# Xharlie/BtcDet

Hardware: AMD Instinct MI355X
Metric: scenes/s fwd+bwd KITTI-Car bs=2/GPU (BtcDet hot path) (higher is better)
Workload: dtype f32

## Files before the change

btcdet_amd/csrc/btc_common.h:

```cpp
#pragma once
#include <hip/hip_runtime.h>
#include <stdint.h>
#include <stdio.h>

#include "../../include/btcdet_hip.h"

#define BTC_EMPTY_KEY (-1)
#define BTC_EMPTY_IDX 0x7F7F7F7F

void btc_set_error(const char* fmt, ...);

#define BTC_CHECK_ARG(cond, ...)            \
  do {                                      \
    if (!(cond)) {                          \
      btc_set_error(__VA_ARGS__);           \
      return BTC_EINVAL;                    \
    }                                       \
  } while (0)

#define BTC_HIP(call)                                                             \
  do {                                                                            \
    hipError_t e_ = (call);                                                       \
    if (e_ != hipSuccess) {                                                       \
      btc_set_error("%s failed: %s (%s:%d)", #call, hipGetErrorString(e_), __FILE__, __LINE__); \
      return BTC_ELAUNCH;                                                         \
    }                                                                             \
  } while (0)

#define BTC_LAUNCH_CHECK()                                                        \
  do {                                                                            \
    hipError_t e_ = hipGetLastError();                                            \
    if (e_ != hipSuccess) {                                                       \
      btc_set_error("kernel launch failed: %s (%s:%d)", hipGetErrorString(e_), __FILE__, __LINE__); \
      return BTC_ELAUNCH;                                                         \
    }                                                                             \
  } while (0)

#if defined(__HIP_DEVICE_COMPILE__) && !defined(__gfx950__)
#error "the fence-free last-arriver protocol (btc_ticket_take) is derived for gfx950's sc1 write-through stores only"
#endif
#if defined(__HIPCC__)
template <class T>
__device__ __forceinline__ void btc_st_agent(T* p, T v) { __hip_atomic_store(p, v, __ATOMIC_RELAXED, __HIP_MEMORY_SCOPE_AGENT); }
template <class T>
__device__ __forceinline__ T btc_ld_agent(const T* p) { return __hip_atomic_load(p, __ATOMIC_RELAXED, __HIP_MEMORY_SCOPE_AGENT); }
__device__ __forceinline__ int btc_ticket_take(int32_t* counter) {
  asm volatile("s_waitcnt vmcnt(0)" ::: "memory");
  return __hip_atomic_fetch_add(counter, 1, __ATOMIC_RELAXED, __HIP_MEMORY_SCOPE_AGENT);
}
__device__ __forceinline__ void btc_ticket_acquire() { __builtin_amdgcn_fence(__ATOMIC_ACQUIRE, "agent"); }
__device__ __forceinline__ bool btc_last_arriver(int32_t* counter, int total) {
  __shared__ int s_last;
  asm volatile("s_waitcnt vmcnt(0)" ::: "memory");
  __syncthreads();
  if (threadIdx.x == 0) s_last = (btc_ticket_take(counter) == total - 1);
  __syncthreads();
  if (!s_last) return false;
  if (threadIdx.x == 0) btc_ticket_acquire();
  __syncthreads();
  return true;
}
#endif

#define BTC_TUNE_KEYS 24
int btc_tune_get(int key);

bool btc_apply_glds_supported(int K, int Cred, int Cres);
bool btc_apply_glds_has_shape(int shape, bool bf = false);
size_t btc_apply_glds_lds_bytes(int shape, int kc, int K, bool bf, int stages = 3);
int btc_apply_glds_stages(int shape, int kc, int K, bool bf, int asked);
int btc_launch_apply_glds(bool trans_w, int shape, int kc, int xcd, bool bf, const void* feat, const float* W, const float* bias,
                          const int32_t* nbr, const int32_t* order , int n_rows, int K, int Cred, int Cres, void* out,
                          hipStream_t stream, const struct BnFuse* bn = nullptr );

int btc_apply(const char* who, int pass, int operands, const void* src, long long src_rows, const void* W, const float* bias, const int32_t* nbr,
              const int32_t* order, int n_rows, int K, int Cin, int Cout, void* dst, hipStream_t stream, const struct BnFuse* bn);

int btc_apply_bf16w(const void* src, const void* Wq, const float* bias, const int32_t* nbr, const int32_t* order, int n_rows, int K, int Cred,
                    int Cres, void* dst, hipStream_t stream, int mirror = 0, const struct BnFuse* bn = nullptr);
constexpr size_t BTC_SCRATCH_HEAD = 64 * 1024;
constexpr long long BTC_SCRATCH_TICKETS = BTC_SCRATCH_HEAD / 4;
void* btc_scratch(hipStream_t stream, size_t* bytes);
struct BnFuse;
int btc_apply_split(const float* src, const void* Ws, const float* bias, const int32_t* nbr, const int32_t* order, int n_rows, int K, int Cred,
                    int Cres, float* dst, hipStream_t stream, int mirror, const BnFuse* bn);

__host__ __device__ __forceinline__ unsigned short btc_f32_to_bf16(float f) {
  union { float f; unsigned u; } c;
  c.f = f;
  unsigned u = c.u;
  if ((u & 0x7fffffffu) > 0x7f800000u) return (unsigned short)((u >> 16) | 0x40);
  u += 0x7fffu + ((u >> 16) & 1u);
  return (unsigned short)(u >> 16);
}
__host__ __device__ __forceinline__ float btc_bf16_to_f32(unsigned short h) {
  union { float f; unsigned u; } c;
  c.u = (unsigned)h << 16;
  return c.f;
}

template <bool BF>
__device__ __forceinline__ float4 btc_ld4(const float* base, size_t i) {
  if (!BF) return *reinterpret_cast<const float4*>(base + i);
  const uint2 v = *reinterpret_cast<const uint2*>(reinterpret_cast<const unsigned short*>(base) + i);
  return make_float4(__uint_as_float(v.x << 16), __uint_as_float(v.x & 0xffff0000u), __uint_as_float(v.y << 16),
                     __uint_as_float(v.y & 0xffff0000u));
}
template <bool BF>
__device__ __forceinline__ float btc_ld1(const float* base, size_t i) {
  if (!BF) return base[i];
  return __uint_as_float((unsigned)reinterpret_cast<const unsigned short*>(base)[i] << 16);
}
template <bool BF>
__device__ __forceinline__ void btc_st4(float* base, size_t i, float a, float b, float c, float d) {
  if (!BF) {
    *reinterpret_cast<float4*>(base + i) = make_float4(a, b, c, d);
  } else {
    uint2 v;
    v.x = (unsigned)btc_f32_to_bf16(a) | ((unsigned)btc_f32_to_bf16(b) << 16);
    v.y = (unsigned)btc_f32_to_bf16(c) | ((unsigned)btc_f32_to_bf16(d) << 16);
    *reinterpret_cast<uint2*>(reinterpret_cast<unsigned short*>(base) + i) = v;
  }
}
template <bool BF>
__device__ __forceinline__ void btc_st1(float* base, size_t i, float a) {
  if (!BF) base[i] = a;
  else reinterpret_cast<unsigned short*>(base)[i] = btc_f32_to_bf16(a);
}

#ifdef __cplusplus
#include <mutex>
constexpr int BTC_MAX_DEVICES = 16;
struct BtcPerDeviceOnce {
  std::once_flag flag[BTC_MAX_DEVICES];
};
template <class F>
static inline void btc_once_per_device(BtcPerDeviceOnce& o, F&& fn) {
  int dev = 0;
  (void)hipGetDevice(&dev);
  std::call_once(o.flag[dev >= 0 && dev < BTC_MAX_DEVICES ? dev : 0], fn);
}
#endif

typedef float f32x4 __attribute__((ext_vector_type(4)));
constexpr int TM = 64;
__host__ __device__ constexpr int ldb_of(int nt) { return nt * 16 + (((nt * 16) % 32 == 0) ? 16 : 0); }

static inline int btc_cdiv(long long a, long long b) { return (int)((a + b - 1) / b); }
static inline size_t btc_align(size_t x, size_t a = 256) { return (x + a - 1) / a * a; }
static inline unsigned btc_pow2_ge(unsigned long long v) {
  unsigned long long p = 1;
  while (p < v) p <<= 1;
  return (unsigned)p;
}

struct BtcCarver {
// ... 35 lines not shown
```

btcdet_amd/csrc/conv_apply_glds.hip:

```cpp
#include "conv_tile.h"

namespace {

__device__ float g_zero_row[64];

constexpr int G_STAGES_DEFAULT = 3;
constexpr int G_STAGES_MAX = 8;

__device__ __forceinline__ void transpose4(const f32x4 v, float& y0, float& y1, float& y2, float& y3) {
  unsigned x0 = __float_as_uint(v[0]), x1 = __float_as_uint(v[1]), x2 = __float_as_uint(v[2]), x3 = __float_as_uint(v[3]);
  auto a = __builtin_amdgcn_permlane32_swap(x0, x2, false, false);
  x0 = a[0]; x2 = a[1];
  auto b = __builtin_amdgcn_permlane32_swap(x1, x3, false, false);
  x1 = b[0]; x3 = b[1];
  auto c = __builtin_amdgcn_permlane16_swap(x0, x1, false, false);
  x0 = c[0]; x1 = c[1];
  auto d = __builtin_amdgcn_permlane16_swap(x2, x3, false, false);
  x2 = d[0]; x3 = d[1];
  y0 = __uint_as_float(x0); y1 = __uint_as_float(x1); y2 = __uint_as_float(x2); y3 = __uint_as_float(x3);
}

template <int WR, int WC, int NTW, bool TRANS_W, int KC, bool BF>
__global__ __launch_bounds__(64 * WR * WC) void conv_apply_g(const void* __restrict__ feat_, const float* __restrict__ W,
                                                             const float* __restrict__ bias, const int32_t* __restrict__ nbr,
// ... 98 lines not shown
      const float* B = (const float*)(ring + st * STAGE + A_BYTES);
      const int aswz = ((wr * 16 + arow) / RPB) & (UPR - 1);
      constexpr int Q = KC / 4;
      constexpr int G = (16 / NTW) < 1 ? 1 : ((16 / NTW) > Q ? Q : (16 / NTW));
      constexpr int NGRP = Q / G;
      float a[2][G], b[2][G][NTW];
      constexpr bool A128 = !BF && (G % 4 == 0);
      constexpr bool B128 = TRANS_W && (G % 4 == 0) && UPB >= 8 && NTW == 1;
      auto load_group = [&](int g, int buf) {
        if (A128) {
#pragma unroll
          for (int jb = 0; jb < G / 4; ++jb) {
            const int u = (g * (G / 4) + jb) * 4 + kq;
            const f32x4 v = *(const f32x4*)(A + ((u ^ aswz) * 16));
            transpose4(v, a[buf][4 * jb], a[buf][4 * jb + 1], a[buf][4 * jb + 2], a[buf][4 * jb + 3]);
          }
        }
        if (B128) {
#pragma unroll
          for (int nt = 0; nt < NTW; ++nt) {
            const float* colp = B + ((wc * NTW + nt) * 16 + arow) * KC;
#pragma unroll
            for (int jb = 0; jb < G / 4; ++jb) {
              const int u = (g * (G / 4) + jb) * 4 + kq;
              const f32x4 v = *(const f32x4*)(colp + ((u ^ (arow & (UPB - 1))) * 4));
              transpose4(v, b[buf][4 * jb][nt], b[buf][4 * jb + 1][nt], b[buf][4 * jb + 2][nt], b[buf][4 * jb + 3][nt]);
            }
          }
        }
#pragma unroll
        for (int i = 0; i < G; ++i) {
          const int q = g * G + i;
          if (A128) {
          } else if (!BF) {
            a[buf][i] = *(const float*)(A + ((q ^ aswz) * 16) + kq * 4);
          } else {
            const unsigned short h = *(const unsigned short*)(A + (((q >> 1) ^ aswz) * 16) + (((q & 1) * 4 + kq) * 2));
            a[buf][i] = __uint_as_float((unsigned)h << 16);
          }
          if (!TRANS_W) {
            const float* bp = B + (q * 4 + kq) * TN + arow;
#pragma unroll
            for (int nt = 0; nt < NTW; ++nt) {
              const int cg = wc * NTW + nt;
              b[buf][i][nt] = bp[((NG >= 2) ? (cg ^ (kq & 1)) : cg) * 16];
            }
          } else if (!B128) {
            const float* bp = B + (wc * NTW * 16 + arow) * KC + (q ^ (arow & (UPB - 1))) * 4 + kq;
#pragma unroll
            for (int nt = 0; nt < NTW; ++nt) b[buf][i][nt] = bp[nt * 16 * KC];
          }
        }
      };
      load_group(0, 0);
#pragma unroll
      for (int g = 0; g < NGRP; ++g) {
        if (g + 1 < NGRP) load_group(g + 1, (g + 1) & 1);
        __builtin_amdgcn_sched_barrier(0);
#pragma unroll
        for (int i = 0; i < G; ++i)
#pragma unroll
          for (int nt = 0; nt < NTW; ++nt)
            acc[nt] = __builtin_amdgcn_mfma_f32_16x16x4f32(a[g & 1][i], b[g & 1][i][nt], acc[nt], 0, 0, 0);
        __builtin_amdgcn_sched_barrier(0);
      }
    }
    st = (st == S - 1) ? 0 : st + 1;
  }

  float vals[NTW][4];
  bool valid[4];
  int rows[4];
#pragma unroll
  for (int r = 0; r < 4; ++r) rows[r] = s_row[wr * 16 + kq * 4 + r];
  const bool ev = !TRANS_W && bn.ev_mean != nullptr;
  typedef typename std::conditional<BF, unsigned short, float>::type OUT;
  apply_tile_epilogue<NTW>(acc, rows, n0 + wc * NTW * 16, bias, Cres, (OUT*)out_, bn, ev, vals, valid);
  if (bn.slots) {
    bn_fuse_wave<NTW>(bn, vals, valid, n0 + wc * NTW * 16, (int)((bx * WR + wr) & (bn.nslots - 1)));
    bn_fuse_finish(bn, (int*)smem, (double*)(smem + 16));
  }
}

template <int WR, int WC, int NTW, bool TRANS_W, int KC, bool BF>
int launch_g(const void* feat, const float* W, const float* bias, const int32_t* nbr, const int32_t* order, int n_rows, int K, int Cred,
             int Cres, void* out, int xcd, hipStream_t stream, const BnFuse& bn) {
  constexpr int TM = 16 * WR, TN = 16 * NTW * WC;
  const int stages = btc_apply_glds_stages(WR * 100 + WC * 10 + NTW, KC, K, BF, (xcd >> APPLY_STAGES_SHIFT) & 15);
  xcd = (xcd & (APPLY_XCD | APPLY_MIRROR)) | (stages << APPLY_STAGES_SHIFT);
  const size_t lds = btc_apply_glds_lds_bytes(WR * 100 + WC * 10 + NTW, KC, K, BF, stages);
  return apply_launch<conv_apply_g<WR, WC, NTW, TRANS_W, KC, BF>>("conv_apply_g", dim3(btc_cdiv(n_rows, TM), Cres / TN), 64 * WR * WC, lds, stream, feat, W,
                                                                  bias, nbr, order, n_rows, K, Cred, Cres, out, xcd,
                                                                  btc_tune_get(BTC_TUNE_APPLY_DEBUG), bn);
}

#define G_ARGS feat, W, bias, nbr, order, n_rows, K, Cred, Cres, out, xcd, stream, bn
#define G_PARAMS                                                                                                             \
  const void *feat, const float *W, const float *bias, const int32_t *nbr, const int32_t *order, int n_rows, int K, int Cred, int Cres, \
      void *out, int xcd, hipStream_t stream, const BnFuse &bn

template <int WR, int WC, int NTW, bool TRANS_W, bool BF>
int launch_g_kc(int kc, G_PARAMS) {
  switch (kc) {
    case 16: return launch_g<WR, WC, NTW, TRANS_W, 16, BF>(G_ARGS);
    case 32: return launch_g<WR, WC, NTW, TRANS_W, 32, BF>(G_ARGS);
    default: return launch_g<WR, WC, NTW, TRANS_W, 64, BF>(G_ARGS);
  }
}

template <bool TRANS_W>
int launch_g_shape(int wr, int wc, int ntw, int kc, bool bf, G_PARAMS) {
  const int code = wr * 100 + wc * 10 + ntw;
  switch (code) {
#define G_CASE2(WR_, WC_, NTW_)                                                      \
  case WR_ * 100 + WC_ * 10 + NTW_:                                                  \
    return bf ? launch_g_kc<WR_, WC_, NTW_, TRANS_W, true>(kc, G_ARGS) : launch_g_kc<WR_, WC_, NTW_, TRANS_W, false>(kc, G_ARGS)
#define G_CASE(WR_, WC_, NTW_)      \
  case WR_ * 100 + WC_ * 10 + NTW_: \
    if (bf) break;                  \
    return launch_g_kc<WR_, WC_, NTW_, TRANS_W, false>(kc, G_ARGS)
    G_CASE2(4, 1, 1); G_CASE(4, 1, 2); G_CASE(4, 1, 4); G_CASE(4, 1, 8);
    G_CASE(4, 2, 1); G_CASE2(4, 2, 2); G_CASE2(4, 2, 4);
    G_CASE2(2, 2, 1); G_CASE(2, 2, 2); G_CASE(2, 2, 4);
    G_CASE(2, 4, 1); G_CASE(2, 4, 2);
    G_CASE2(1, 4, 1); G_CASE(1, 4, 2);
#undef G_CASE
#undef G_CASE2
    default: break;
  }
  btc_set_error("conv_apply_g: no instance for WR=%d WC=%d NTW=%d bf16=%d", wr, wc, ntw, (int)bf);
  return BTC_EINVAL;
}

}

bool btc_apply_glds_has_shape(int shape, bool bf) {
  static const int shapes[] = {411, 412, 414, 418, 421, 422, 424, 221, 222, 224, 241, 242, 141, 142};
  static const int shapes_bf[] = {411, 422, 424, 221, 141};
  if (bf) {
    for (int v : shapes_bf)
      if (v == shape) return true;
    return false;
  }
  for (int v : shapes)
    if (v == shape) return true;
  return false;
}

size_t btc_apply_glds_lds_bytes(int shape, int kc, int K, bool bf, int stages) {
  const int tm = 16 * (shape / 100), tn = 16 * ((shape / 10) % 10) * (shape % 10);
  const size_t a_bytes = ((size_t)tm * kc * (bf ? 2 : 4) + 1023) / 1024 * 1024;
  return (size_t)(stages > 0 ? stages : G_STAGES_DEFAULT) * (a_bytes + (size_t)kc * tn * 4) + apply_tail_bytes(tm, K);
}

int btc_apply_glds_stages(int shape, int kc, int K, bool bf, int asked) {
  const int tm = 16 * (shape / 100), tn = 16 * ((shape / 10) % 10) * (shape % 10), nw = (shape / 100) * ((shape / 10) % 10);
  const size_t a_bytes = ((size_t)tm * kc * (bf ? 2 : 4) + 1023) / 1024 * 1024, stage = a_bytes + (size_t)kc * tn * 4;
  const int npi = (int)(((a_bytes / 1024) + nw - 1) / nw + ((size_t)kc * tn / 256 + nw - 1) / nw);
  int s = asked ? asked : btc_tune_get(BTC_TUNE_APPLY_STAGES);
  if (!s) {
    s = (int)((size_t)48 * 1024 / stage);
    if (s > 6) s = 6;
  }
  if (s < 3) s = 3;
  if (s > G_STAGES_MAX) s = G_STAGES_MAX;
  while (s > 3 && ((s - 2) * npi > 63 || btc_apply_glds_lds_bytes(shape, kc, K, bf, s) > 160 * 1024)) --s;
  return s;
}

bool btc_apply_glds_supported(int K, int Cred, int Cres) { return K <= 64 && Cred % 16 == 0 && Cres % 16 == 0 && Cred >= 16; }

int btc_launch_apply_glds(bool trans_w, int shape, int kc, int xcd, bool bf, const void* feat, const float* W, const float* bias,
                          const int32_t* nbr, const int32_t* order, int n_rows, int K, int Cred, int Cres, void* out, hipStream_t stream,
                          const BnFuse* bn_) {
  if (n_rows <= 0) return BTC_OK;
  const BnFuse bn = bn_ ? *bn_ : btc_bn_fuse_none();
  const int wr = shape / 100, wc = (shape / 10) % 10, ntw = shape % 10;
  BTC_CHECK_ARG(btc_apply_glds_supported(K, Cred, Cres) && wc * ntw > 0 && Cres % (16 * wc * ntw) == 0 && Cred % kc == 0 &&
                    (kc == 16 || kc == 32 || kc == 64),
                "conv_apply_g: unsupported K=%d Cred=%d Cres=%d shape=%d kc=%d", K, Cred, Cres, shape, kc);
  return trans_w ? launch_g_shape<true>(wr, wc, ntw, kc, bf, G_ARGS) : launch_g_shape<false>(wr, wc, ntw, kc, bf, G_ARGS);
}
```

btcdet_amd/csrc/sparse_conv.hip:

```cpp
#include "conv_tile.h"

namespace {

constexpr int KC = 32;
constexpr int LDA = KC + 2;

template <int NT, bool TRANS_W, bool VEC, int KB, int THREADS>
__global__ __launch_bounds__(THREADS) void conv_apply(const float* __restrict__ feat, const float* __restrict__ W,
                                                  const float* __restrict__ bias, const int32_t* __restrict__ nbr,
                                                  int n_rows, int K, int Cred, int Cres, float* __restrict__ out, int mirror, const BnFuse bn) {
  extern __shared__ __attribute__((aligned(16))) char smem[];
  constexpr int TM = THREADS / 4;
  constexpr int LDB = ldb_of(NT);
  constexpr int NB = NT * 512 / THREADS;
  float* As = (float*)smem;
  float* Bs = As + KB * TM * LDA;
  int32_t* s_nbr = (int32_t*)(Bs + KB * KC * LDB);
  int32_t* s_kact = s_nbr + TM * K;
  int32_t* s_nact = s_kact + K;

  const int tid = threadIdx.x, lane = tid & 63, wave = tid >> 6;
  const int row0 = blockIdx.x * TM;
  const int n0 = blockIdx.y * (NT * 16);

// ... 251 lines not shown
    constexpr bool ev = EV;
#pragma unroll
    for (int r = 0; r < 4; ++r) valid[r] = row0 + kq * 4 + r < n_rows;
#pragma unroll
    for (int nt = 0; nt < NT; ++nt) {
      const int col = nt * 16 + lrow;
      const float bv0 = (bias && col < Cres) ? bias[col] : 0.f;
      BnEvalCol ec = {0.f, 0.f, 1.f, 0.f};
      if (ev) ec = bn_eval_col(bn, col);
#pragma unroll
      for (int r = 0; r < 4; ++r) {
        const int row = row0 + kq * 4 + r;
        vals[nt][r] = bias ? (acc[nt][r] + bv0) : acc[nt][r];
        if (ev) vals[nt][r] = bn_affine(vals[nt][r], ec.m, ec.rs, ec.g, ec.b, bn.ev_relu);
        if (col < Cres && row < n_rows) out[(size_t)row * Cres + col] = vals[nt][r];
      }
    }
    if (bn.slots) bn_fuse_wave<NT>(bn, vals, valid, 0, (int)(tile & (bn.nslots - 1)));
    __builtin_amdgcn_wave_barrier();
  }
  if (bn.slots) bn_fuse_finish(bn, (int*)smem, (double*)(smem + 16));
}


__global__ __launch_bounds__(256) void maxpool_fwd_k(const float* __restrict__ feat, const int32_t* __restrict__ nbr,
                                                     int n_out, int K, int C, float* __restrict__ out) {
  long long t = (long long)blockIdx.x * blockDim.x + threadIdx.x;
  if (t >= (long long)n_out * C) return;
  int i = (int)(t / C), c = (int)(t % C);
  float m = 0.f;
  for (int k = 0; k < K; ++k) {
    int j = nbr[(size_t)i * K + k];
    if (j >= 0) m = fmaxf(m, feat[(size_t)j * C + c]);
  }
  out[t] = m;
}

__global__ __launch_bounds__(256) void maxpool_bwd_k(const float* __restrict__ feat, const float* __restrict__ out,
                                                     const float* __restrict__ dout, const int32_t* __restrict__ nbr_in,
                                                     int n_in, int K, int C, float* __restrict__ din) {
  long long t = (long long)blockIdx.x * blockDim.x + threadIdx.x;
  if (t >= (long long)n_in * C) return;
  int j = (int)(t / C), c = (int)(t % C);
  float v = feat[t], g = 0.f;
  for (int k = 0; k < K; ++k) {
    int i = nbr_in[(size_t)j * K + k];
    if (i >= 0 && out[(size_t)i * C + c] == v) g += dout[(size_t)i * C + c];
  }
  din[t] = g;
}

__global__ __launch_bounds__(256) void dense_fwd_k(const float* __restrict__ feat, const int4* __restrict__ idx, int n, int C,
                                                   int D, int H, int Wd, float* __restrict__ dense) {
  long long t = (long long)blockIdx.x * blockDim.x + threadIdx.x;
  if (t >= (long long)n * C) return;
  int c = (int)(t / n), i = (int)(t % n);
  int4 q = idx[i];
  size_t vol = (size_t)D * H * Wd;
  dense[((size_t)q.x * C + c) * vol + ((size_t)q.y * H + q.z) * Wd + q.w] = feat[(size_t)i * C + c];
}

__global__ __launch_bounds__(256) void dense_bwd_k(const float* __restrict__ ddense, const int4* __restrict__ idx, int n, int C,
                                                   int D, int H, int Wd, float* __restrict__ dfeat) {
  long long t = (long long)blockIdx.x * blockDim.x + threadIdx.x;
  if (t >= (long long)n * C) return;
  int c = (int)(t / n), i = (int)(t % n);
  int4 q = idx[i];
  size_t vol = (size_t)D * H * Wd;
  dfeat[(size_t)i * C + c] = ddense[((size_t)q.x * C + c) * vol + ((size_t)q.y * H + q.z) * Wd + q.w];
}

template <int NT, bool TRANS_W, int THREADS>
int launch_apply_t(dim3 grid, size_t lds, hipStream_t stream, bool vec, const float* feat, const float* W, const float* bias,
                   const int32_t* nbr, int n_rows, int K, int Cred, int Cres, float* out, int mirror, const BnFuse& bn) {
  if (vec) return apply_launch<conv_apply<NT, TRANS_W, true, 1, THREADS>>("conv_apply", grid, THREADS, lds, stream, feat, W, bias, nbr, n_rows, K, Cred, Cres, out, mirror, bn);
  return apply_launch<conv_apply<NT, TRANS_W, false, 1, THREADS>>("conv_apply", grid, THREADS, lds, stream, feat, W, bias, nbr, n_rows, K, Cred, Cres, out, mirror, bn);
}

template <bool TRANS_W, bool EV>
int launch_ws(int nt, int wgs, size_t lds, hipStream_t stream, const float* feat, const float* W, const float* bias, const int32_t* nbr, int n_rows,
              int K, int Cred, int Cres, float* out, int mirror, const BnFuse& bn) {
  if (nt == 1) return apply_launch<conv_apply_ws<1, TRANS_W, EV>>("conv_apply_ws", wgs, WS_WAVES * 64, lds, stream, feat, W, bias, nbr, n_rows, K, Cred, Cres, out, mirror, bn);
  return apply_launch<conv_apply_ws<2, TRANS_W, EV>>("conv_apply_ws", wgs, WS_WAVES * 64, lds, stream, feat, W, bias, nbr, n_rows, K, Cred, Cres, out, mirror, bn);
}

template <bool TRANS_W>
int launch_apply(const float* feat, const float* W, const float* bias, const int32_t* nbr, int n_rows, int K, int Cred,
                 int Cres, float* out, hipStream_t stream, bool bf = false, const int32_t* order = nullptr, int mirror = 0,
                 const BnFuse* bn_ = nullptr) {
  const BnFuse bn = bn_ ? *bn_ : btc_bn_fuse_none();
  if (n_rows <= 0) return BTC_OK;
  BTC_CHECK_ARG(!bf || btc_apply_glds_supported(K, Cred, Cres),
                "bf16 activations need channel counts that are multiples of 16 (K=%d, %d -> %d): convert to fp32", K, Cred, Cres);
  int nt = Cres <= 16 ? 1 : (Cres <= 32 ? 2 : (Cres <= 64 ? 4 : 8));
  const int t_kernel = btc_tune_get(BTC_TUNE_APPLY_KERNEL), t_nt = btc_tune_get(BTC_TUNE_APPLY_NT);
  if (bf || (t_kernel != 1 && btc_apply_glds_supported(K, Cred, Cres) && (t_kernel == 2 || n_rows < 100000 || (Cred >= 64 && Cres >= 64)))) {
    int shape, kc = (Cred % 64 == 0) ? 64 : ((Cred % 32 == 0) ? 32 : 16);
    if (bf) {
      if (Cres % 128 == 0) shape = 424;
      else if (Cres % 64 == 0) shape = n_rows < 8192 ? 141 : 422;
      else if (Cres % 32 == 0) shape = 221;
      else shape = 411;
    } else if (Cres % 128 == 0) {
      shape = n_rows < 7000 ? 222 : (n_rows < 13000 ? 242 : (n_rows <= 16384 ? 424 : (n_rows < 19500 ? 242 : 424)));
    } else if (Cres % 64 == 0) {
      if (kc == 64) shape = n_rows < 11000 ? 141 : 241;
      else shape = n_rows < 13000 ? 141 : 222;
    } else if (Cres % 32 == 0) {
      shape = 221;
    } else {
      shape = 411;
    }
    if (t_nt > 8 && !bf) {
      int wc = (t_nt / 10) % 10, ntw = t_nt % 10;
      while (ntw > 1 && Cres % (16 * wc * ntw)) ntw >>= 1;
      while (wc > 1 && Cres % (16 * wc * ntw)) wc >>= 1;
      const int cand = (t_nt / 100) * 100 + wc * 10 + ntw;
      if (btc_apply_glds_has_shape(cand)) shape = cand;
    }
    const int t_kc = btc_tune_get(BTC_TUNE_APPLY_KC);
    if (t_kc && Cred % t_kc == 0) kc = t_kc;
    while (kc > 16 && btc_apply_glds_lds_bytes(shape, kc, K, bf) > 160 * 1024) kc >>= 1;
    return btc_launch_apply_glds(TRANS_W, shape, kc, apply_flags(mirror), bf, feat, W, bias, nbr, order, n_rows, K, Cred, Cres, out, stream, &bn);
  }
  if (t_kernel != 1 && Cred <= 4 * WS_Q && Cres <= 32 && K <= 64 && n_rows >= 2048 && ws_lds_bytes(K, Cred, nt) <= 160 * 1024) {
    const int n_tiles16 = btc_cdiv(n_rows, 16);
    int wgs = btc_cdiv(n_tiles16, WS_WAVES);
    if (wgs > 256) wgs = 256;
    size_t lds = ws_lds_bytes(K, Cred, nt);
    if (bn.slots && lds < 16 + (size_t)16 * WS_WAVES * 64) lds = 16 + (size_t)16 * WS_WAVES * 64;
    if constexpr (!TRANS_W) {
      if (bn.ev_mean) return launch_ws<false, true>(nt, wgs, lds, stream, feat, W, bias, nbr, n_rows, K, Cred, Cres, out, mirror, bn);
    }
    return launch_ws<TRANS_W, false>(nt, wgs, lds, stream, feat, W, bias, nbr, n_rows, K, Cred, Cres, out, mirror, bn);
  }
  const int tm = 64;
  const int n_tiles = btc_cdiv(n_rows, tm);
  while (nt > 2 && (long long)n_tiles * btc_cdiv(Cres, nt * 16) < 512) nt >>= 1;
  if (t_nt && t_nt <= 8) nt = t_nt;
  dim3 grid(n_tiles, btc_cdiv(Cres, nt * 16));
  size_t lds = (size_t)(tm * LDA + KC * ldb_of(nt)) * sizeof(float) + (size_t)(tm * K + K + 1) * sizeof(int32_t);
  const bool vec = (Cred & 3) == 0;
#define BTC_APPLY(NT_) launch_apply_t<NT_, TRANS_W, 256>(grid, lds, stream, vec, feat, W, bias, nbr, n_rows, K, Cred, Cres, out, mirror, bn)
  switch (nt) {
    case 1: return BTC_APPLY(1);
    case 2: return BTC_APPLY(2);
    case 4: return BTC_APPLY(4);
    default: return BTC_APPLY(8);
  }
#undef BTC_APPLY
}

int split_source_ok(const char* who, long long src_rows, int Cred) {
  BTC_CHECK_ARG(src_rows >= 0, "%s: BTC_OPERANDS_F32_SPLIT needs the row count of src (btc_conv_apply_src / btc_conv_bn_relu_fwd_src)", who);
  BTC_CHECK_ARG(src_rows * Cred * 4 < 0xFFFFFF00LL, "%s: a source of %lld rows x %d channels is past the 32-bit gather offsets of the split-operand "
                "kernel (4 GB): use BTC_OPERANDS_F32", who, src_rows, Cred);
  return BTC_OK;
}

}

int btc_apply(const char* who, int pass, int operands, const void* src, long long src_rows, const void* W, const float* bias, const int32_t* nbr,
              const int32_t* order, int n_rows, int K, int Cin, int Cout, void* dst, hipStream_t stream, const BnFuse* bn) {
  BTC_CHECK_ARG((pass == BTC_PASS_FWD || pass == BTC_PASS_DGRAD || pass == BTC_PASS_DGRAD_MIRROR) && operands >= BTC_OPERANDS_F32 &&
                    operands <= BTC_OPERANDS_F32_SPLIT, "%s: pass=%d operands=%d", who, pass, operands);
  const int mirror = pass == BTC_PASS_DGRAD_MIRROR;
  const bool fwd = pass == BTC_PASS_FWD;
  BTC_CHECK_ARG(K <= BTC_CONV_K_MAX, "%s: K=%d offsets, more than BTC_CONV_K_MAX = %d", who, K, BTC_CONV_K_MAX);
  BTC_CHECK_ARG(K >= 1 && Cin >= 1 && Cout >= 1 && n_rows >= 0, "%s: bad sizes", who);
  BTC_CHECK_ARG(fwd || bias == nullptr, "%s: dgrad takes no bias", who);
  BTC_CHECK_ARG(!bn || Cout <= BN_FUSE_CMAX, "%s: more than %d channels", who, BN_FUSE_CMAX);
  const int Cred = fwd ? Cin : Cout, Cres = fwd ? Cout : Cin;
  if (operands == BTC_OPERANDS_BF16) {
    const bool ok = btc_conv_bf16w_supported(K, Cred, Cres);
    if (bn) BTC_CHECK_ARG(ok, "%s: bf16 operands need K <= 64, Cin %% 32 == 0, Cout %% 16 == 0", who);
    else BTC_CHECK_ARG(ok, "%s: bf16 operands need K <= 64, Cred %% 32 == 0, Cres %% 16 == 0 (K=%d, %d -> %d)", who, K, Cin, Cout);
    return btc_apply_bf16w(src, W, bias, nbr, order, n_rows, K, Cred, Cres, dst, stream, mirror, bn);
  }
  if (operands == BTC_OPERANDS_F32_SPLIT) {
    if (n_rows > 0) {
      const int rc = split_source_ok(who, src_rows, Cred);
      if (rc) return rc;
    }
    return btc_apply_split((const float*)src, W, bias, nbr, order, n_rows, K, Cred, Cres, (float*)dst, stream, mirror, bn);
  }
  const bool bf = operands == BTC_OPERANDS_BF16_ACT;
  if (fwd) return launch_apply<false>((const float*)src, (const float*)W, bias, nbr, n_rows, K, Cred, Cres, (float*)dst, stream, bf, order, 0, bn);
  return launch_apply<true>((const float*)src, (const float*)W, nullptr, nbr, n_rows, K, Cred, Cres, (float*)dst, stream, bf, order, mirror, bn);
}

#define BTC_SIZES_OK(who, n) BTC_CHECK_ARG(K >= 1 && Cin >= 1 && Cout >= 1 && (n) >= 0, who ": bad sizes")

extern "C" int btc_conv_fwd(const float* feat, const float* W, const float* bias, const int32_t* nbr_out, int n_out, int K,
                            int Cin, int Cout, float* out, void* stream) {
  BTC_SIZES_OK("btc_conv_fwd", n_out);
  return btc_apply("btc_conv_fwd", BTC_PASS_FWD, BTC_OPERANDS_F32, feat, -1LL, W, bias, nbr_out, nullptr, n_out, K, Cin, Cout, out, (hipStream_t)stream, nullptr);
}

extern "C" int btc_conv_dgrad(const float* dout, const float* W, const int32_t* nbr_in, int n_in, int K, int Cin, int Cout,
                              float* din, void* stream) {
  BTC_SIZES_OK("btc_conv_dgrad", n_in);
  return btc_apply("btc_conv_dgrad", BTC_PASS_DGRAD, BTC_OPERANDS_F32, dout, -1LL, W, nullptr, nbr_in, nullptr, n_in, K, Cin, Cout, din, (hipStream_t)stream, nullptr);
}

extern "C" int btc_conv_fwd_bf16(const void* feat, const float* W, const float* bias, const int32_t* nbr_out, int n_out, int K,
                                 int Cin, int Cout, void* out, void* stream) {
// ... 73 lines not shown
```

include/btcdet_hip.h:

```cpp
#ifndef BTCDET_HIP_H
#define BTCDET_HIP_H

#include <stddef.h>
#include <stdint.h>

#ifdef __cplusplus
extern "C" {
#endif

#define BTC_OK 0
#define BTC_EINVAL (-1)
#define BTC_ELAUNCH (-2)
#define BTC_ERANGE (-3)

#define BTC_MODE_SUBM 0
#define BTC_MODE_CONV 1
#define BTC_MODE_TRANSPOSE 2

const char* btc_last_error(void);
int btc_version(void);

#define BTC_TUNE_APPLY_KERNEL 0
#define BTC_TUNE_APPLY_NT 1
#define BTC_TUNE_APPLY_XCD 2
#define BTC_TUNE_APPLY_KC 4
#define BTC_TUNE_WGRAD_PH 5
#define BTC_TUNE_WGRAD_WGS 6
#define BTC_TUNE_POV_SELECT 7
#define BTC_TUNE_BF16_OPERANDS 8
#define BTC_TUNE_BN_FWD_KB 9
#define BTC_TUNE_BN_BWD_KB 10
#define BTC_TUNE_WGRAD_PIPE 11
#define BTC_TUNE_BN_FUSE 12
#define BTC_TUNE_SPLIT_Z 15
#define BTC_TUNE_SPLIT_LOADERS 17
#define BTC_TUNE_SPLIT 14
#define BTC_TUNE_APPLY_STAGES 13
#define BTC_TUNE_WGRAD_X 18
#define BTC_TUNE_WGRAD_X_DEPTH 20
#define BTC_TUNE_RB_MARK_MULTI 19
#define BTC_TUNE_SPLIT_PAIR 21
#define BTC_TUNE_WGRAD_NARROW 22
#define BTC_TUNE_EVAL_FOLD 23
#define BTC_TUNE_APPLY_DEBUG 3
int btc_tune_set(int key, int value);
int btc_tune_value(int key);

size_t btc_voxelize_ws_bytes(int n, int batch, int max_points);
int btc_voxelize(const float* points, int n, int ld, int xyz_col, int feat_col, int C,
                 const int32_t* scene_offsets, int batch, const float* h_range, const float* h_vsize,
                 const int32_t* h_grid, int max_points, int max_voxels, float* voxels, int32_t* coords,
                 int32_t* num, int32_t* d_total, void* ws, size_t ws_bytes, void* stream);

int btc_cart_to_occ_coords(const float* in, float* out, int n, int ld, int mode, void* stream);

int btc_voxel_shift_col(float* voxels, const int32_t* coords, int m, int max_points, int C, int col,
                        const float* rot_by_batch, float sign, void* stream);

size_t btc_range_mask_ws_bytes(int n);
int btc_range_mask_compact(const float* points, const float* points_b, int n, int ld, int ld_b, const int32_t* scene_offsets, int batch,
                           const float* h_range_xyxy, float* out, float* out_b, int32_t* out_offsets, int32_t* keep_idx, void* ws,
                           size_t ws_bytes, void* stream);
int btc_gather_rows(const float* src, const int32_t* idx, int n_out, int ld, int n_src, float* out, int32_t* bad_count, void* stream);

int btc_out_shape(const int32_t* h_in_shape, const int32_t* h_k, const int32_t* h_s, const int32_t* h_p,
                  const int32_t* h_d, const int32_t* h_outpad, int mode, int32_t* h_out_shape);

size_t btc_rulebook_subm_ws_bytes(int n);
int btc_rulebook_subm(const int32_t* indices, int n, int batch, const int32_t* h_shape, const int32_t* h_k,
                      const int32_t* h_d, int32_t* nbr_out, int32_t* nbr_in, void* ws, size_t ws_bytes,
                      void* stream);

size_t btc_rulebook_conv_ws_bytes(int batch, const int32_t* h_out_shape);
int btc_rulebook_conv_count(const int32_t* indices, int n, int batch, const int32_t* h_in_shape,
                            const int32_t* h_out_shape, const int32_t* h_k, const int32_t* h_s,
                            const int32_t* h_p, const int32_t* h_d, int mode, int32_t* d_n_out, void* ws,
                            size_t ws_bytes, void* stream);
int btc_rulebook_conv_fill(const int32_t* indices, int n, int batch, const int32_t* h_in_shape,
                           const int32_t* h_out_shape, const int32_t* h_k, const int32_t* h_s,
                           const int32_t* h_p, const int32_t* h_d, int mode, int n_out, int32_t* out_indices,
                           int32_t* nbr_out, int32_t* nbr_in, void* ws, size_t ws_bytes, void* stream);

#define BTC_CHAIN_MAX_LAYERS 32
typedef struct BtcChainLayer {
  int32_t kind, ref, mode;
  int32_t in_shape[3], out_shape[3], k[3], s[3], p[3], d[3];
} BtcChainLayer;
size_t btc_chain_ws_bytes(const BtcChainLayer* h_layers, int n_layers, int batch, int n0);
int btc_chain_caps(const BtcChainLayer* h_layers, int n_layers, int batch, int n0, int64_t* h_cap);
int btc_chain_levels(const int32_t* indices, int n0, int batch, const BtcChainLayer* h_layers, int n_layers,
                     int32_t* const* h_out_indices, const int64_t* h_cap, int32_t* d_counts, void* ws, size_t ws_bytes, void* stream);
int btc_chain_maps(const int32_t* indices, int n0, int batch, const BtcChainLayer* h_layers, int n_layers, const int32_t* h_counts,
                   int32_t* const* h_out_indices, int32_t* const* h_nbr_out, int32_t* const* h_nbr_in,
                   int32_t* const* h_first_out ,
                   int32_t* const* h_first_in , void* ws, size_t ws_bytes, void* stream);

size_t btc_pairs_from_nbr_ws_bytes(int n_out, int K);
int btc_pairs_from_nbr(const int32_t* nbr_out, int n_out, int K, int n_in, int32_t* pairs, int32_t* pair_num, void* ws,
                       size_t ws_bytes, void* stream);

int btc_conv_fwd(const float* feat, const float* W, const float* bias , const int32_t* nbr_out,
                 int n_out, int K, int Cin, int Cout, float* out, void* stream);
int btc_conv_dgrad(const float* dout, const float* W, const int32_t* nbr_in, int n_in, int K, int Cin,
                   int Cout, float* din, void* stream);
size_t btc_conv_wgrad_ws_bytes(int n_out, int K, int Cin, int Cout, int n_in);
int btc_conv_wgrad(const float* feat, const float* dout, const int32_t* nbr_out, int n_out, const int32_t* nbr_in,
                   int n_in, int K, int Cin, int Cout, float* dW, void* ws, size_t ws_bytes, void* stream);

int btc_conv_fwd_bf16(const void* feat, const float* W, const float* bias, const int32_t* nbr_out, int n_out, int K, int Cin,
                      int Cout, void* out, void* stream);
int btc_conv_dgrad_bf16(const void* dout, const float* W, const int32_t* nbr_in, int n_in, int K, int Cin, int Cout,
                        void* din, void* stream);
int btc_conv_wgrad_bf16(const void* feat, const void* dout, const int32_t* nbr_out, int n_out, const int32_t* nbr_in,
                        int n_in, int K, int Cin, int Cout, float* dW, void* ws, size_t ws_bytes, void* stream);

int btc_conv_bf16w_supported(int K, int Cred, int Cres);
int btc_weights_to_bf16(const float* W, int K, int Cin, int Cout, void* w_bf16, void* wt_bf16, void* stream);
int btc_weights_to_bf16_multi(const float* const* W, void* const* w_bf16, void* const* wt_bf16, const int32_t* K, const int32_t* Cin,
                              const int32_t* Cout, int n, void* stream);
int btc_conv_fwd_bf16w(const void* feat, const void* wt_bf16, const float* bias, const int32_t* nbr_out, int n_out, int K, int Cin,
                       int Cout, void* out, void* stream);
int btc_conv_dgrad_bf16w(const void* dout, const void* w_bf16, const int32_t* nbr_in, int n_in, int K, int Cin, int Cout, void* din,
                         void* stream);

// ... 209 lines not shown
```

Before: 583.8.

## Batch several kernel offsets per pipeline item in gather-LDS conv apply

Adds a conv_apply_gk kernel variant in which each pipeline stage loads KB kernel offsets' activation rows and weights at once when the reduced channel count fits in a single chunk (Cred == kc ≤ 32, fp32 activations). The aim is to cut the number of per-item waits and barriers and to give each stage more MFMA work for narrow-channel layers. By default it picks KB=4 for kc=16 and KB=2 for kc=32 on the supported tile shapes, and a new tune key can override this. The cost is larger LDS stages, which may lower occupancy or the number of stages, plus extra template instances.

Result: no change. 582.1 (-0.3%).

```diff
diff --git a/btcdet_amd/csrc/btc_common.h b/btcdet_amd/csrc/btc_common.h
--- a/btcdet_amd/csrc/btc_common.h
+++ b/btcdet_amd/csrc/btc_common.h
@@ -67,11 +67,13 @@
 
 bool btc_apply_glds_supported(int K, int Cred, int Cres);
 bool btc_apply_glds_has_shape(int shape, bool bf = false);
-size_t btc_apply_glds_lds_bytes(int shape, int kc, int K, bool bf, int stages = 3);
-int btc_apply_glds_stages(int shape, int kc, int K, bool bf, int asked);
+bool btc_apply_glds_has_kb(int shape, int kc, int kb);
+size_t btc_apply_glds_lds_bytes(int shape, int kc, int K, bool bf, int stages = 3, int kb = 1);
+int btc_apply_glds_stages(int shape, int kc, int K, bool bf, int asked, int kb = 1);
 int btc_launch_apply_glds(bool trans_w, int shape, int kc, int xcd, bool bf, const void* feat, const float* W, const float* bias,
                           const int32_t* nbr, const int32_t* order , int n_rows, int K, int Cred, int Cres, void* out,
-                          hipStream_t stream, const struct BnFuse* bn = nullptr );
+                          hipStream_t stream, const struct BnFuse* bn = nullptr ,
+                          int kb = 1 );
 
 int btc_apply(const char* who, int pass, int operands, const void* src, long long src_rows, const void* W, const float* bias, const int32_t* nbr,
               const int32_t* order, int n_rows, int K, int Cin, int Cout, void* dst, hipStream_t stream, const struct BnFuse* bn);
diff --git a/btcdet_amd/csrc/conv_apply_glds.hip b/btcdet_amd/csrc/conv_apply_glds.hip
--- a/btcdet_amd/csrc/conv_apply_glds.hip
+++ b/btcdet_amd/csrc/conv_apply_glds.hip
@@ -204,13 +204,219 @@
   }
 }
 
-template <int WR, int WC, int NTW, bool TRANS_W, int KC, bool BF>
+template <int WR, int WC, int NTW, bool TRANS_W, int KC, bool BF, int KB>
+__global__ __launch_bounds__(64 * WR * WC) void conv_apply_gk(const void* __restrict__ feat_, const float* __restrict__ W,
+                                                             const float* __restrict__ bias, const int32_t* __restrict__ nbr,
+                                                             const int32_t* __restrict__ order, int n_rows, int K, int Cred, int Cres,
+                                                             void* __restrict__ out_, int flags, int dbg, const BnFuse bn) {
+  extern __shared__ __attribute__((aligned(16))) char smem[];
+  const int S = ((flags >> APPLY_STAGES_SHIFT) & 15) ? ((flags >> APPLY_STAGES_SHIFT) & 15) : G_STAGES_DEFAULT;
+  constexpr int NW = WR * WC, THREADS = 64 * NW;
+  constexpr int TM = 16 * WR, TN = 16 * NTW * WC, NG = NTW * WC;
+  constexpr int ES = BF ? 2 : 4;
+  constexpr int KW = KB * KC;
+  static_assert(KW <= 64 && (KB == 1 || !BF), "an item is 64 channels at most; several offsets per item: fp32 activations");
+  constexpr int UPR = KW * ES / 16;
+  constexpr int UPS = KC * ES / 16;
+  constexpr int UPB = KW / 4;
+  constexpr int RPB = (128 / (KW * ES)) < 1 ? 1 : (128 / (KW * ES));
+  constexpr int A_UNITS = TM * UPR;
+  constexpr int NAI_TOTAL = (A_UNITS + 63) / 64;
+  constexpr int NAI = (NAI_TOTAL + NW - 1) / NW;
+  constexpr int NBI_TOTAL = KW * TN / 256;
+  constexpr int NBI = (NBI_TOTAL + NW - 1) / NW;
+  constexpr int NPI = NAI + NBI;
+  constexpr int A_BYTES = (TM * KW * ES + 1023) / 1024 * 1024;
+  constexpr int STAGE = A_BYTES + KW * TN * 4;
+  char* ring = smem;
+  APPLY_TAIL(ring + S * STAGE, TM, K);
+  const char* feat = (const char*)feat_;
+
+  const int tid = threadIdx.x, lane = tid & 63, wave = tid >> 6;
+  const int wr = wave / WC, wc = wave % WC;
+  const ApplyTile tile = apply_tile_prologue<TM, THREADS>(s_nbr, s_kact, s_nact, s_row, nbr, order, n_rows, K, flags, wr);
+  const int bx = tile.bx, n0 = blockIdx.y * TN, n_act = tile.n_act;
+  const unsigned long long wave_act = tile.wave_act;
+  const int n_chunks = Cred / KC;
+  const int n_items = (dbg & 32) ? 0 : (KB > 1 ? (n_act + KB - 1) / KB : n_act * n_chunks);
+  if (dbg & 16) return;
+  f32x4 acc[NTW];
+#pragma unroll
+  for (int nt = 0; nt < NTW; ++nt) acc[nt] = (f32x4){0.f, 0.f, 0.f, 0.f};
+
+  int iq = 0, ir = 0, cq = 0, cr = 0;
+  auto issue = [&](int st) {
+    const int k = s_kact[iq];
+    const int cc = ir * KC;
+    const int ib = iq, last = n_act - 1;
+    if constexpr (KB > 1) iq += KB;
+    else if (++ir == n_chunks) { ir = 0; ++iq; }
+    char* As = ring + st * STAGE;
+    float* Bs = (float*)(As + A_BYTES);
+#pragma unroll
+    for (int t = 0; t < NAI; ++t) {
+      if (dbg & 8) break;
+      const int ai = (wave + NW * t) % NAI_TOTAL;
+      const int U = ai * 64 + lane;
+      if (A_UNITS % 64 == 0 || U < A_UNITS) {
+        const int rloc = U / UPR;
+        const int uw = (U % UPR) ^ ((rloc / RPB) & (UPR - 1));
+        const int e = ib + uw / UPS, u = uw % UPS;
+        int nb;
+        if constexpr (KB == 1) nb = s_nbr[rloc * K + k];
+        else nb = e <= last ? s_nbr[rloc * K + s_kact[e]] : -1;
+        const char* src = nb >= 0 ? feat + ((size_t)nb * Cred + cc) * ES + u * 16 : (const char*)g_zero_row;
+        glds16(src, As + ai * 1024);
+      }
+    }
+    const float* Wk1 = W + (size_t)k * Cred * Cres;
+#pragma unroll
+    for (int t = 0; t < NBI; ++t) {
+      if (dbg & 4) break;
+      const int ii = (wave + NW * t) % NBI_TOTAL;
+      const int U = ii * 64 + lane;
+      const float* src;
+      if (!TRANS_W) {
+        const int kw = U / (TN / 4), pu = U % (TN / 4);
+        const int e = ib + kw / KC, kr = kw % KC;
+        const float* Wk = KB == 1 ? Wk1 : W + (size_t)s_kact[e <= last ? e : last] * Cred * Cres;
+        const int g = (NG >= 2) ? ((pu >> 2) ^ (kr & 1)) : (pu >> 2);
+        src = Wk + (size_t)(cc + kr) * Cres + n0 + g * 16 + (pu & 3) * 4;
+      } else {
+        const int c = U / UPB, pu = U % UPB;
+        const int rw = pu ^ (c & (UPB - 1));
+        const int e = ib + rw / (KC / 4), ru = rw % (KC / 4);
+        const float* Wk = KB == 1 ? Wk1 : W + (size_t)s_kact[e <= last ? e : last] * Cred * Cres;
+        src = Wk + (size_t)(n0 + c) * Cred + cc + ru * 4;
+      }
+      glds16(src, Bs + ii * 256);
+    }
+  };
+
+  const int arow = lane & 15, kq = lane >> 4;
+#define WAIT_ITEMS(n) wait_vm<((n) * NPI > 63 ? 63 : (n) * NPI)>()
+  for (int i = 0; i < S - 1 && i < n_items; ++i) issue(i);
+  int st = 0;
+  for (int item = 0; item < n_items; ++item) {
+    const int left = n_items - 1 - item, fl = left < S - 2 ? left : S - 2;
+    switch (fl) {
+      case 0: wait_vm<0>(); break;
+      case 1: WAIT_ITEMS(1); break;
+      case 2: WAIT_ITEMS(2); break;
+      case 3: WAIT_ITEMS(3); break;
+      case 4: WAIT_ITEMS(4); break;
+      case 5: WAIT_ITEMS(5); break;
+      default: WAIT_ITEMS(6); break;
+    }
+#undef WAIT_ITEMS
+    __builtin_amdgcn_s_barrier();
+    asm volatile("" ::: "memory");
+    if (item + S - 1 < n_items && !(dbg & 2)) issue(st == 0 ? S - 1 : st - 1);
+    const int k0 = s_kact[cq], cb = cq;
+    if constexpr (KB > 1) cq += KB;
+    else if (++cr == n_chunks) { cr = 0; ++cq; }
+#pragma unroll
+    for (int sb = 0; sb < KB; ++sb) {
+      if (KB > 1 && cb + sb >= n_act) break;
+      const int k = sb == 0 ? k0 : s_kact[cb + sb];
+      if (((wave_act >> k) & 1ull) && !(dbg & 1)) {
+        const char* A = ring + st * STAGE + (wr * 16 + arow) * (KW * ES);
+        const float* B = (const float*)(ring + st * STAGE + A_BYTES);
+        const int aswz = ((wr * 16 + arow) / RPB) & (UPR - 1);
+        const int ua = sb * UPS, ub = sb * (KC / 4);
+        constexpr int Q = KC / 4;
+        constexpr int G = (16 / NTW) < 1 ? 1 : ((16 / NTW) > Q ? Q : (16 / NTW));
+        constexpr int NGRP = Q / G;
+        float a[2][G], b[2][G][NTW];
+        constexpr bool A128 = !BF && (G % 4 == 0);
+        constexpr bool B128 = TRANS_W && (G % 4 == 0) && UPB >= 8 && NTW == 1;
+        auto load_group = [&](int g, int buf) {
+          if (A128) {
+#pragma unroll
+            for (int jb = 0; jb < G / 4; ++jb) {
+              const int u = (g * (G / 4) + jb) * 4 + kq;
+              const f32x4 v = *(const f32x4*)(A + (((ua + u) ^ aswz) * 16));
+              transpose4(v, a[buf][4 * jb], a[buf][4 * jb + 1], a[buf][4 * jb + 2], a[buf][4 * jb + 3]);
+            }
+          }
+          if (B128) {
+#pragma unroll
+            for (int nt = 0; nt < NTW; ++nt) {
+              const float* colp = B + ((wc * NTW + nt) * 16 + arow) * KW;
+#pragma unroll
+              for (int jb = 0; jb < G / 4; ++jb) {
+                const int u = (g * (G / 4) + jb) * 4 + kq;
+                const f32x4 v = *(const f32x4*)(colp + (((ub + u) ^ (arow & (UPB - 1))) * 4));
+                transpose4(v, b[buf][4 * jb][nt], b[buf][4 * jb + 1][nt], b[buf][4 * jb + 2][nt], b[buf][4 * jb + 3][nt]);
+              }
+            }
+          }
+#pragma unroll
+          for (int i = 0; i < G; ++i) {
+            const int q = g * G + i;
+            if (A128) {
+            } else if (!BF) {
+              a[buf][i] = *(const float*)(A + (((ua + q) ^ aswz) * 16) + kq * 4);
+            } else {
+              const unsigned short h = *(const unsigned short*)(A + (((ua + (q >> 1)) ^ aswz) * 16) + (((q & 1) * 4 + kq) * 2));
+              a[buf][i] = __uint_as_float((unsigned)h << 16);
+            }
+            if (!TRANS_W) {
+              const float* bp = B + (sb * KC + q * 4 + kq) * TN + arow;
+#pragma unroll
+              for (int nt = 0; nt < NTW; ++nt) {
+                const int cg = wc * NTW + nt;
+                b[buf][i][nt] = bp[((NG >= 2) ? (cg ^ (kq & 1)) : cg) * 16];
+              }
+            } else if (!B128) {
+              const float* bp = B + (wc * NTW * 16 + arow) * KW + ((ub + q) ^ (arow & (UPB - 1))) * 4 + kq;
+#pragma unroll
+              for (int nt = 0; nt < NTW; ++nt) b[buf][i][nt] = bp[nt * 16 * KW];
+            }
+          }
+        };
+        load_group(0, 0);
+#pragma unroll
+        for (int g = 0; g < NGRP; ++g) {
+          if (g + 1 < NGRP) load_group(g + 1, (g + 1) & 1);
+          __builtin_amdgcn_sched_barrier(0);
+#pragma unroll
+          for (int i = 0; i < G; ++i)
+#pragma unroll
+            for (int nt = 0; nt < NTW; ++nt)
+              acc[nt] = __builtin_amdgcn_mfma_f32_16x16x4f32(a[g & 1][i], b[g & 1][i][nt], acc[nt], 0, 0, 0);
+          __builtin_amdgcn_sched_barrier(0);
+        }
+      }
+    }
+    st = (st == S - 1) ? 0 : st + 1;
+  }
+
+  float vals[NTW][4];
+  bool valid[4];
+  int rows[4];
+#pragma unroll
+  for (int r = 0; r < 4; ++r) rows[r] = s_row[wr * 16 + kq * 4 + r];
+  const bool ev = !TRANS_W && bn.ev_mean != nullptr;
+  typedef typename std::conditional<BF, unsigned short, float>::type OUT;
+  apply_tile_epilogue<NTW>(acc, rows, n0 + wc * NTW * 16, bias, Cres, (OUT*)out_, bn, ev, vals, valid);
+  if (bn.slots) {
+    bn_fuse_wave<NTW>(bn, vals, valid, n0 + wc * NTW * 16, (int)((bx * WR + wr) & (bn.nslots - 1)));
+    bn_fuse_finish(bn, (int*)smem, (double*)(smem + 16));
+  }
+}
+
+template <int WR, int WC, int NTW, bool TRANS_W, int KC, bool BF, int KB = 1>
 int launch_g(const void* feat, const float* W, const float* bias, const int32_t* nbr, const int32_t* order, int n_rows, int K, int Cred,
              int Cres, void* out, int xcd, hipStream_t stream, const BnFuse& bn) {
   constexpr int TM = 16 * WR, TN = 16 * NTW * WC;
-  const int stages = btc_apply_glds_stages(WR * 100 + WC * 10 + NTW, KC, K, BF, (xcd >> APPLY_STAGES_SHIFT) & 15);
+  const int stages = btc_apply_glds_stages(WR * 100 + WC * 10 + NTW, KC, K, BF, (xcd >> APPLY_STAGES_SHIFT) & 15, KB);
   xcd = (xcd & (APPLY_XCD | APPLY_MIRROR)) | (stages << APPLY_STAGES_SHIFT);
-  const size_t lds = btc_apply_glds_lds_bytes(WR * 100 + WC * 10 + NTW, KC, K, BF, stages);
+  const size_t lds = btc_apply_glds_lds_bytes(WR * 100 + WC * 10 + NTW, KC, K, BF, stages, KB);
+  if constexpr (KB > 1)
+    return apply_launch<conv_apply_gk<WR, WC, NTW, TRANS_W, KC, BF, KB>>("conv_apply_gk", dim3(btc_cdiv(n_rows, TM), Cres / TN), 64 * WR * WC, lds, stream, feat, W,
+                                                                         bias, nbr, order, n_rows, K, Cred, Cres, out, xcd,
+                                                                         btc_tune_get(BTC_TUNE_APPLY_DEBUG), bn);
   return apply_launch<conv_apply_g<WR, WC, NTW, TRANS_W, KC, BF>>("conv_apply_g", dim3(btc_cdiv(n_rows, TM), Cres / TN), 64 * WR * WC, lds, stream, feat, W,
                                                                   bias, nbr, order, n_rows, K, Cred, Cres, out, xcd,
                                                                   btc_tune_get(BTC_TUNE_APPLY_DEBUG), bn);
@@ -230,9 +436,23 @@
   }
 }
 
+template <int WR, int WC, int NTW, bool TRANS_W>
+int launch_g_kb(int kc, int kb, G_PARAMS) {
+  if (kc == 16 && kb == 2) return launch_g<WR, WC, NTW, TRANS_W, 16, false, 2>(G_ARGS);
+  if (kc == 16 && kb == 4) return launch_g<WR, WC, NTW, TRANS_W, 16, false, 4>(G_ARGS);
+  return launch_g<WR, WC, NTW, TRANS_W, 32, false, 2>(G_ARGS);
+}
+
 template <bool TRANS_W>
-int launch_g_shape(int wr, int wc, int ntw, int kc, bool bf, G_PARAMS) {
+int launch_g_shape(int wr, int wc, int ntw, int kc, bool bf, int kb, G_PARAMS) {
   const int code = wr * 100 + wc * 10 + ntw;
+  if (kb > 1) {
+    switch (code) {
+      case 411: return launch_g_kb<4, 1, 1, TRANS_W>(kc, kb, G_ARGS);
+      case 221: return launch_g_kb<2, 2, 1, TRANS_W>(kc, kb, G_ARGS);
+      default: return launch_g_kb<1, 4, 1, TRANS_W>(kc, kb, G_ARGS);
+    }
+  }
   switch (code) {
 #define G_CASE2(WR_, WC_, NTW_)                                                      \
   case WR_ * 100 + WC_ * 10 + NTW_:                                                  \
@@ -269,13 +489,20 @@
   return false;
 }
 
-size_t btc_apply_glds_lds_bytes(int shape, int kc, int K, bool bf, int stages) {
+bool btc_apply_glds_has_kb(int shape, int kc, int kb) {
+  if (kb == 1) return true;
+  return (shape == 411 || shape == 221 || shape == 141) && ((kc == 16 && (kb == 2 || kb == 4)) || (kc == 32 && kb == 2));
+}
+
+size_t btc_apply_glds_lds_bytes(int shape, int kc, int K, bool bf, int stages, int kb) {
+  kc *= kb;
   const int tm = 16 * (shape / 100), tn = 16 * ((shape / 10) % 10) * (shape % 10);
   const size_t a_bytes = ((size_t)tm * kc * (bf ? 2 : 4) + 1023) / 1024 * 1024;
   return (size_t)(stages > 0 ? stages : G_STAGES_DEFAULT) * (a_bytes + (size_t)kc * tn * 4) + apply_tail_bytes(tm, K);
 }
 
-int btc_apply_glds_stages(int shape, int kc, int K, bool bf, int asked) {
+int btc_apply_glds_stages(int shape, int kc, int K, bool bf, int asked, int kb) {
+  kc *= kb;
   const int tm = 16 * (shape / 100), tn = 16 * ((shape / 10) % 10) * (shape % 10), nw = (shape / 100) * ((shape / 10) % 10);
   const size_t a_bytes = ((size_t)tm * kc * (bf ? 2 : 4) + 1023) / 1024 * 1024, stage = a_bytes + (size_t)kc * tn * 4;
   const int npi = (int)(((a_bytes / 1024) + nw - 1) / nw + ((size_t)kc * tn / 256 + nw - 1) / nw);
@@ -294,12 +521,14 @@
 
 int btc_launch_apply_glds(bool trans_w, int shape, int kc, int xcd, bool bf, const void* feat, const float* W, const float* bias,
                           const int32_t* nbr, const int32_t* order, int n_rows, int K, int Cred, int Cres, void* out, hipStream_t stream,
-                          const BnFuse* bn_) {
+                          const BnFuse* bn_, int kb) {
   if (n_rows <= 0) return BTC_OK;
   const BnFuse bn = bn_ ? *bn_ : btc_bn_fuse_none();
+  BTC_CHECK_ARG(kb == 1 || (!bf && Cred == kc && btc_apply_glds_has_kb(shape, kc, kb)), "conv_apply_g: no instance with %d offsets per item (shape=%d kc=%d Cred=%d bf16=%d)",
+                kb, shape, kc, Cred, (int)bf);
   const int wr = shape / 100, wc = (shape / 10) % 10, ntw = shape % 10;
   BTC_CHECK_ARG(btc_apply_glds_supported(K, Cred, Cres) && wc * ntw > 0 && Cres % (16 * wc * ntw) == 0 && Cred % kc == 0 &&
                     (kc == 16 || kc == 32 || kc == 64),
                 "conv_apply_g: unsupported K=%d Cred=%d Cres=%d shape=%d kc=%d", K, Cred, Cres, shape, kc);
-  return trans_w ? launch_g_shape<true>(wr, wc, ntw, kc, bf, G_ARGS) : launch_g_shape<false>(wr, wc, ntw, kc, bf, G_ARGS);
-}
+  return trans_w ? launch_g_shape<true>(wr, wc, ntw, kc, bf, kb, G_ARGS) : launch_g_shape<false>(wr, wc, ntw, kc, bf, kb, G_ARGS);
+}
diff --git a/btcdet_amd/csrc/sparse_conv.hip b/btcdet_amd/csrc/sparse_conv.hip
--- a/btcdet_amd/csrc/sparse_conv.hip
+++ b/btcdet_amd/csrc/sparse_conv.hip
@@ -357,6 +357,11 @@
               int K, int Cred, int Cres, float* out, int mirror, const BnFuse& bn) {
   if (nt == 1) return apply_launch<conv_apply_ws<1, TRANS_W, EV>>("conv_apply_ws", wgs, WS_WAVES * 64, lds, stream, feat, W, bias, nbr, n_rows, K, Cred, Cres, out, mirror, bn);
   return apply_launch<conv_apply_ws<2, TRANS_W, EV>>("conv_apply_ws", wgs, WS_WAVES * 64, lds, stream, feat, W, bias, nbr, n_rows, K, Cred, Cres, out, mirror, bn);
+}
+
+int apply_glds_kb_policy(int kc, int shape) {
+  if (kc == 16) return (shape == 411 || shape == 221) ? 4 : 1;
+  return (shape == 221 || shape == 141) ? 2 : 1;
 }
 
 template <bool TRANS_W>
@@ -396,7 +401,13 @@
     const int t_kc = btc_tune_get(BTC_TUNE_APPLY_KC);
     if (t_kc && Cred % t_kc == 0) kc = t_kc;
     while (kc > 16 && btc_apply_glds_lds_bytes(shape, kc, K, bf) > 160 * 1024) kc >>= 1;
-    return btc_launch_apply_glds(TRANS_W, shape, kc, apply_flags(mirror), bf, feat, W, bias, nbr, order, n_rows, K, Cred, Cres, out, stream, &bn);
+    int kb = 1;
+    if (!bf && Cred == kc && kc <= 32) {
+      const int t_kb = btc_tune_get(BTC_TUNE_APPLY_KB);
+      kb = t_kb > 0 ? t_kb : apply_glds_kb_policy(kc, shape);
+      while (kb > 1 && (!btc_apply_glds_has_kb(shape, kc, kb) || btc_apply_glds_lds_bytes(shape, kc, K, bf, 3, kb) > 160 * 1024)) kb >>= 1;
+    }
+    return btc_launch_apply_glds(TRANS_W, shape, kc, apply_flags(mirror), bf, feat, W, bias, nbr, order, n_rows, K, Cred, Cres, out, stream, &bn, kb);
   }
   if (t_kernel != 1 && Cred <= 4 * WS_Q && Cres <= 32 && K <= 64 && n_rows >= 2048 && ws_lds_bytes(K, Cred, nt) <= 160 * 1024) {
     const int n_tiles16 = btc_cdiv(n_rows, 16);
diff --git a/include/btcdet_hip.h b/include/btcdet_hip.h
--- a/include/btcdet_hip.h
+++ b/include/btcdet_hip.h
@@ -40,6 +40,7 @@
 #define BTC_TUNE_WGRAD_X_DEPTH 20
 #define BTC_TUNE_RB_MARK_MULTI 19
 #define BTC_TUNE_SPLIT_PAIR 21
+#define BTC_TUNE_APPLY_KB 16
 #define BTC_TUNE_WGRAD_NARROW 22
 #define BTC_TUNE_EVAL_FOLD 23
 #define BTC_TUNE_APPLY_DEBUG 3
```
